# mazrk7/gmvae

Hardware: AMD Instinct MI355X
Metric: ELBO-samples/sec (higher is better)
Workload: dtype f32; 1 GPU; gmvae train step (noise+fwd+bwd+allreduce+TF-Adam), D=784 K=10 L=64 hidden=[64] S=1, batch 1024/GPU x 1 GPU (BASELINE configs[2]); global_batch=1024, parallelism=dp1, hipgraph=True, input_pipeline_on_device=False, safe_schedule=False

## Files before the change

gmvae_amd/csrc/mega2.hpp:

```cpp
#pragma once
#include "mega.hpp"

namespace gmvae {

struct M2 {
  static constexpr int H = 64, L = 64, K = 10, KP = 16, L2 = 128, D = 784, K2 = 12;
  static constexpr int NT = D / 16;
  static constexpr int DC = 16 * kM2ProdTiles;
  static constexpr int b_y0 = 0, b_y1 = 64, b_g0 = 80, b_p = 144, b_g1 = 272, b_d0 = 400;
  static constexpr int Wy1f = 512;
  static constexpr int Wg0yf = Wy1f + 1024;
  static constexpr int Wpf = Wg0yf + 1024;
  static constexpr int imgF_early = Wpf + 2048;
  static constexpr int Wg1f = imgF_early;
  static constexpr int Wd0f = Wg1f + 8192;
  static constexpr int imgF = Wd0f + 4096;
  static constexpr int Wd0b = 0;
  static constexpr int Wg1b = Wd0b + 4096;
  static constexpr int Wg0yb = Wg1b + 8192;
  static constexpr int Wpb = Wg0yb + 1024;
  static constexpr int Wy1b = Wpb + 2048;
  static constexpr int imgB = Wy1b + 1024;
  static constexpr int dF = 0, dFq = 16 * DC * 4;
  static constexpr int dB = 4 * dFq, dBq = (DC / 4) * 64 * 4;
  static constexpr int dbias = dB + 4 * dBq, dbq = DC;
  static constexpr int dimg = dbias + 4 * dbq;
  static constexpr int ld64 = 68, ld128 = 132, ldk = 20;
  static constexpr int IMG = 0;
  static constexpr int P_h1 = IMG + imgF;
  static constexpr int P_y = P_h1 + 16 * ld128;
  static constexpr int P_hg = P_y + 16 * ldk;
  static constexpr int P_pp = P_hg + 16 * ld64;
  static constexpr int P_qp = P_pp + 16 * ld128;
  static constexpr int P_z = P_qp + 16 * ld128;
  static constexpr int P_sp = P_z + 16 * ld64;
  static constexpr int P_hd = P_sp + 16 * 64;
  static constexpr int P_eps = P_hd + 16 * ld64;
  static constexpr int P_u = P_eps + 16 * 64;
  static constexpr int P_lg = P_u + 256;
  static constexpr int nll = P_lg + 16 * ldk;
  static constexpr int rsum = nll + 64;
  static constexpr int red = rsum + 128;
  static constexpr int dred = red + 2048;
  static constexpr int P_dhd = dred + 8192;
  static constexpr int total = P_dhd + 16 * ld64;
  static constexpr int P_dz = dred;
  static constexpr int P_dqp = P_dz + 16 * ld64;
  static constexpr int P_dpp = P_dqp + 16 * ld128;
  static constexpr int P_dhg = P_dpp + 16 * ld128;
  static constexpr int P_dl = P_dhg + 16 * ld64;
  static_assert(P_dl + 16 * ldk <= P_dhd, "backward panels must fit the dred region");
  static_assert(total * 4 <= 160 * 1024, "LDS budget");
  static constexpr int fl_kq = 196, fl_W = imgF, fl_A = fl_W + fl_kq * 64;
  static_assert(fl_A + 32 * kFlLda <= total, "first-layer staging must fit");
  static constexpr int imgF_pieces = (imgF + 2047) / 2048;
};

template <int KT, int NPAD>
__device__ __forceinline__ f32x4 m2_tile(const float* __restrict__ Wimg, const int nt, const float* __restrict__ Pin,
                                         const int ld, const int kt0, const int ln, const int lk, f32x4 acc) {
  float4 a[KT], b[KT];
#pragma unroll
  for (int t = 0; t < KT; ++t) {
    a[t] = *reinterpret_cast<const float4*>(Wimg + ((((kt0 + t) * 4 + lk) * NPAD + nt * 16 + ln) << 2));
    b[t] = *reinterpret_cast<const float4*>(Pin + ln * ld + (kt0 + t) * 16 + 4 * lk);
  }
#pragma unroll
  for (int t = 0; t < KT; ++t) {
    acc = __builtin_amdgcn_mfma_f32_16x16x4f32(a[t].x, b[t].x, acc, 0, 0, 0);
    acc = __builtin_amdgcn_mfma_f32_16x16x4f32(a[t].y, b[t].y, acc, 0, 0, 0);
    acc = __builtin_amdgcn_mfma_f32_16x16x4f32(a[t].z, b[t].z, acc, 0, 0, 0);
    acc = __builtin_amdgcn_mfma_f32_16x16x4f32(a[t].w, b[t].w, acc, 0, 0, 0);
  }
  return acc;
}
__device__ __forceinline__ void granule_publish(unsigned long long* p, const unsigned long long v) {
  __hip_atomic_store(p, v, __ATOMIC_RELAXED, __HIP_MEMORY_SCOPE_AGENT);
}
typedef unsigned u32x4_t __attribute__((ext_vector_type(4)));
__device__ __forceinline__ void granule2_publish(unsigned long long* p, const unsigned epoch, const float v0, const float v1) {
  const u32x4_t t = {__float_as_uint(v0), epoch, __float_as_uint(v1), epoch};
  asm volatile("global_store_dwordx4 %0, %1, off sc1\n\ts_nop 1" ::"v"(p), "v"(t) : "memory");
}
__device__ __forceinline__ u32x4_t granule2_load(const unsigned long long* p) {
  u32x4_t r;
  asm volatile("global_load_dwordx4 %0, %1, off sc1" : "=v"(r) : "v"(p) : "memory");
  return r;
}
#ifndef M2_L2_SWEEPS
#define M2_L2_SWEEPS 0
#endif
__device__ __forceinline__ u32x4_t granule2_load_l2(const unsigned long long* p) {
  u32x4_t r;
  asm volatile("global_load_dwordx4 %0, %1, off sc0" : "=v"(r) : "v"(p) : "memory");
  return r;
}
template <int N>
__device__ __forceinline__ void g2_wait(u32x4_t (&v)[N]) {
  static_assert(N == 6 || N == 8, "operand lists below");
  if constexpr (N == 8)
    asm volatile("s_waitcnt vmcnt(0)" : "+v"(v[0]), "+v"(v[1]), "+v"(v[2]), "+v"(v[3]), "+v"(v[4]), "+v"(v[5]), "+v"(v[6]), "+v"(v[7])::"memory");
  else
    asm volatile("s_waitcnt vmcnt(0)" : "+v"(v[0]), "+v"(v[1]), "+v"(v[2]), "+v"(v[3]), "+v"(v[4]), "+v"(v[5])::"memory");
}
__device__ __forceinline__ float4 f4(const f32x4 v) { return make_float4(v[0], v[1], v[2], v[3]); }
__device__ __forceinline__ float4 ld4(const float* p) { return *reinterpret_cast<const float4*>(p); }
__device__ __forceinline__ void st4(float* p, const float4 v) { *reinterpret_cast<float4*>(p) = v; }
__device__ __forceinline__ void st1o(float* p, const float v) {
  __hip_atomic_store(reinterpret_cast<unsigned*>(p), __float_as_uint(v), __ATOMIC_RELAXED, __HIP_MEMORY_SCOPE_AGENT);
}

template <int FUSE>
__device__ __forceinline__ int mega2_body(const MegaArgs& a, float* const sm, unsigned* const m3_flags = nullptr) {
  constexpr int H = M2::H, L = M2::L, K = M2::K, D = M2::D, L2 = M2::L2, K2 = M2::K2;
  constexpr int Q = 4, H2f = 2 * H;
  const int tid = threadIdx.x, lane = tid & 63, wave = __builtin_amdgcn_readfirstlane(tid >> 6);
  const int ln = lane & 15, lk = lane >> 4;
  const int B = a.B, nP = ((B + kPanel - 1) / kPanel + 1) & ~1;
  const int bid = blockIdx.x;
  const int q = bid < nP * (Q - 1) ? 1 + bid / nP : 0;
  const int pnl = bid < nP * (Q - 1) ? bid % nP : bid - nP * (Q - 1);
  const int r0 = pnl * kPanel;
  const int nrow = min(kPanel, B - r0);
  const bool lead = q == 0;
  const bool act = FUSE ? q == 1 : lead;
  if (a.span && tid == 0) a.span[2 * bid] = wall_clock64();
#define M2_SPAN_END() if (!FUSE && a.span && threadIdx.x == 0) a.span[2 * blockIdx.x + 1] = wall_clock64()
  const unsigned spin_limit = *a.err_word ? 0u : (1u << 19);
  const unsigned epoch0 = *a.epoch_word;
  float* const img = sm + M2::IMG;
  float *P_h1 = sm + M2::P_h1, *P_y = sm + M2::P_y, *P_hg = sm + M2::P_hg, *P_pp = sm + M2::P_pp, *P_qp = sm + M2::P_qp;
  float *P_z = sm + M2::P_z, *P_sp = sm + M2::P_sp, *P_hd = sm + M2::P_hd, *P_eps = sm + M2::P_eps, *P_u = sm + M2::P_u;
  float *P_lg = sm + M2::P_lg, *nllp = sm + M2::nll, *rsum = sm + M2::rsum, *red = sm + M2::red, *dred = sm + M2::dred;
  float* P_dhd = sm + M2::P_dhd;
  GMVAE_STAMP(0);
#define M2_WC(i) if (a.dbg && a.fine == 5 && threadIdx.x == 0) a.dbg[(size_t)blockIdx.x * 16 + 8 + (i)] = wall_clock64()
#define M2_FC(i) if (a.dbg && a.fine == 6 && threadIdx.x == 0) a.dbg[(size_t)blockIdx.x * 16 + 8 + (i)] = __builtin_amdgcn_s_memtime()

  float flt[4] = {0.f, 0.f, 0.f, 0.f};
  {
    constexpr int KQ = M2::fl_kq, kq4 = KQ / 4;
    float* const Wst = sm + M2::fl_W;
    float* const A_x = sm + M2::fl_A;
    const int k0 = q * KQ;
    const int sp = pnl >> 1, hh = pnl & 1;
    const int rs0 = sp * 2 * kPanel;
    const float* const W0 = (hh ? a.w0b : a.w0a) + (long long)k0 * H;
    const unsigned epoch_fl = epoch0;
    const unsigned long long step = a.step_dev[0];
    constexpr int qer = L / 4, qur = (K + 3) / 4, qe = kPanel * qer, qu = kPanel * qur;
    float nz[4] = {0.f, 0.f, 0.f, 0.f};
    f32x4 acc = {0.f, 0.f, 0.f, 0.f};
    unsigned xw[4];
    const int row_ = lane >> 4, piece = lane & 15;
    const int src = row_ * 64 + ((piece ^ ((row_ & 1) << 2)) << 2);
#pragma unroll
    for (int j = 0; j < 3; ++j) {
      const int idx = wave + 8 * j;
      __builtin_amdgcn_global_load_lds(W0 + (idx << 8) + src, Wst + (idx << 8), 16, 0, 0);
    }
#pragma unroll
    for (int it = 0; it < 4; ++it) {
      const int i = min(tid + it * kMT, 2 * kPanel * kq4 - 1);
      const int row = i / kq4, k4 = (i - row * kq4) * 4;
      const unsigned wv = *reinterpret_cast<const unsigned*>(a.x + (long long)min(rs0 + row, B - 1) * D + k0 + k4);
      xw[it] = rs0 + row < B ? wv : 0u;
    }
#pragma unroll
    for (int j = 0; j < 4; ++j) {
      const int idx = 24 + min(wave + 8 * j, 24);
      __builtin_amdgcn_global_load_lds(W0 + (idx << 8) + src, Wst + (idx << 8), 16, 0, 0);
    }
#pragma unroll
    for (int j = 0; j < M2::imgF_pieces; ++j) {
      const int c = min(wave * 256 + j * 2048, M2::imgF - 256);
      __builtin_amdgcn_global_load_lds(a.img2f + c + lane * 4, img + c, 16, 0, 0);
    }
    M2_FC(0);
    if (tid < qe + qu && nrow > 0) {
      const bool is_u = tid >= qe;
      const int li = is_u ? tid - qe : tid;
      const int qpr = is_u ? qur : qer;
      const int row = li / qpr, quad = li - row * qpr;
      noise_vals(a.row0 + (unsigned long long)(r0 + row), (unsigned)quad, is_u, a.seed, step, nz);
    }
    static_assert(M2::imgF_pieces == 9, "the counted waits below assume 9 image pieces per wave");
    asm volatile("s_waitcnt vmcnt(13)" ::: "memory");
    M2_FC(1);
#pragma unroll
    for (int it = 0; it < 4; ++it) {
      const int i = tid + it * kMT;
      if (i < 2 * kPanel * kq4) {
        const int row = i / kq4, k4 = (i - row * kq4) * 4;
        const unsigned w = xw[it];
        float2* const dst = reinterpret_cast<float2*>(A_x + row * kFlLda + k4);
        dst[0] = make_float2((float)(w & 0xff), (float)((w >> 8) & 0xff));
        dst[1] = make_float2((float)((w >> 16) & 0xff), (float)(w >> 24));
      }
    }
    __syncthreads();
    M2_FC(2);
    const int tl = wave & 3, rt = wave >> 2;
    const int swz = ((tl * 16 + ln) ^ ((lk & 1) << 4)) - (tl * 16 + ln);
    const float* const Wt = Wst + swz;
    const float* const At = A_x + rt * kPanel * kFlLda;
    acc = tile_ksteps<1, kFlLda>(At, Wt, H, 1, tl, 0, 24, 24, lane, acc);
    M2_FC(3);
    asm volatile("s_waitcnt vmcnt(9)" ::: "memory");
    __syncthreads();
    M2_FC(4);
    acc = tile_ksteps<1, kFlLda>(At, Wt, H, 1, tl, 24, 49, 49, lane, acc);
    constexpr int ngr = 2 * kPanel * H;
    {
      unsigned long long* xo = a.xfl + (((long long)sp * 4 + q) * 2 + hh) * ngr;
      granule2_publish(xo + ((wave * 2 + 0) * 64 + lane) * 2, epoch_fl, acc[0], acc[1]);
      granule2_publish(xo + ((wave * 2 + 1) * 64 + lane) * 2, epoch_fl, acc[2], acc[3]);
    }
    M2_FC(5);
    if (bid == 0 && tid == 0) a.step_dev[1] = step;
    if (nrow <= 0) {
      asm volatile("s_waitcnt vmcnt(0)" ::: "memory");
      M2_SPAN_END();
      return 0;
    }
    M2_WC(5);
    __syncthreads();
    if (tid < qe) {
      st4(P_eps + tid * 4, make_float4(nz[0], nz[1], nz[2], nz[3]));
    } else if (tid < qe + qu) {
      const int li = tid - qe, row = li / qur, k0u = (li - row * qur) * 4;
#pragma unroll
      for (int j = 0; j < 4; ++j)
        if (k0u + j < K) P_u[row * 16 + k0u + j] = nz[j];
    }
    {
      const unsigned long long* const xp0 = a.xfl + ((long long)sp * 4 * 2 + (wave >> 2)) * ngr + (((hh * 4 + (wave & 3)) * 2) * 64 + lane) * 2;
      u32x4_t gv[8];
      unsigned spins = 0;
      for (;;) {
        if (M2_L2_SWEEPS > 0 && spins < M2_L2_SWEEPS && (wave >> 2) == hh) {
#pragma unroll
          for (int pq = 0; pq < 4; ++pq) {
            gv[2 * pq] = granule2_load_l2(xp0 + (long long)pq * 2 * ngr);
            gv[2 * pq + 1] = granule2_load_l2(xp0 + (long long)pq * 2 * ngr + 128);
          }
        } else {
#pragma unroll
          for (int pq = 0; pq < 4; ++pq) {
            gv[2 * pq] = granule2_load(xp0 + (long long)pq * 2 * ngr);
            gv[2 * pq + 1] = granule2_load(xp0 + (long long)pq * 2 * ngr + 128);
          }
        }
        g2_wait(gv);
        bool ok = true;
#pragma unroll
        for (int i = 0; i < 8; ++i) ok = ok && gv[i][1] == epoch_fl && gv[i][3] == epoch_fl;
        if (__all(ok)) break;
        if (++spins > spin_limit) {
          if (lane == 0) atomicExch(a.err_word, 1u);
#pragma unroll
          for (int i = 0; i < 8; ++i) { gv[i][0] = 0x7fc00000u; gv[i][2] = 0x7fc00000u; }
          break;
        }
        __builtin_amdgcn_s_sleep(2);
      }
#pragma unroll
      for (int r = 0; r < 4; ++r) {
        flt[r] = __uint_as_float(gv[0 + (r >> 1)][2 * (r & 1)]);
        flt[r] += __uint_as_float(gv[2 + (r >> 1)][2 * (r & 1)]);
        flt[r] += __uint_as_float(gv[4 + (r >> 1)][2 * (r & 1)]);
        flt[r] += __uint_as_float(gv[6 + (r >> 1)][2 * (r & 1)]);
      }
      if (a.dbg && a.fine >= 5 && tid == 0) {
        a.dbg[(size_t)blockIdx.x * 16 + 14] = spins;
        a.dbg[(size_t)blockIdx.x * 16 + 0] = __builtin_amdgcn_s_getreg((3 << 11) | 20) & 15u;
      }
    }
  }
  M2_WC(6);
  M2_FC(6);
  const int ntq = m2_dec_ntiles(q);
  const bool two = wave + 8 < ntq;
  const bool one = wave < ntq;
  float4 wf[2][4], wb[2][4], bias4[2];
  unsigned xb[2] = {0u, 0u};
  {
    const float* const dfq = a.dimg2 + M2::dF + q * M2::dFq;
    const float* const dbq = a.dimg2 + M2::dB + q * M2::dBq;
    const float* const bq = a.dimg2 + M2::dbias + q * M2::dbq;
#pragma unroll
    for (int it = 0; it < 2; ++it) {
      if (it == 0 ? one : two) {
        const int lt = wave + 8 * it;
#pragma unroll
        for (int kt = 0; kt < 4; ++kt) wf[it][kt] = ld4(dfq + (((kt * 4 + lk) * M2::DC + lt * 16 + ln) << 2));
#pragma unroll
        for (int ht = 0; ht < 4; ++ht) wb[it][ht] = ld4(dbq + (((lt * 4 + lk) * 64 + ht * 16 + ln) << 2));
        bias4[it] = ld4(bq + lt * 16 + 4 * lk);
        const int c0 = m2_dec_tile(q, lt) * 16;
        xb[it] = *reinterpret_cast<const unsigned*>(a.x + (long long)min(r0 + ln, B - 1) * D + c0 + 4 * lk);
      }
    }
  }
  if (two) asm volatile("s_waitcnt vmcnt(20)" ::: "memory");
  else if (one) asm volatile("s_waitcnt vmcnt(10)" ::: "memory");
  else asm volatile("s_waitcnt vmcnt(0)" ::: "memory");
  __syncthreads();
  M2_FC(7);
  {
#pragma unroll
    for (int r = 0; r < 4; ++r) {
      const int row = lk * 4 + r, col = wave * 16 + ln;
      if (col < H) {
        const float h = fmaxf(flt[r] + img[M2::b_y0 + col], 0.f);
        P_h1[row * M2::ld128 + col] = h;
      } else {
        P_h1[row * M2::ld128 + col] = flt[r];
      }
    }
  }
  __syncthreads();
  GMVAE_STAMP(1);
  if (act && tid < 256) {
    const int row = tid >> 4, c = (tid & 15) << 2;
    if (row < nrow) st4o(a.hy1 + (long long)(r0 + row) * H + c, ld4(P_h1 + row * M2::ld128 + c));
  }
  if (wave < 4) {
    f32x4 acc = {0.f, 0.f, 0.f, 0.f};
    acc = m2_tile<1, 16>(img + M2::Wy1f, 0, P_h1, M2::ld128, wave, ln, lk, acc);
    st4(red + wave * 320 + ln * M2::ldk + 4 * lk, f4(acc));
  }
  __syncthreads();
  if (tid < 256) {
    const int row = tid >> 4, k = tid & 15;
    const bool ok = row < nrow, kv = k < K;
    float lg = -INFINITY, av = -INFINITY;
    if (kv) {
      lg = red[row * M2::ldk + k] + red[320 + row * M2::ldk + k] + red[640 + row * M2::ldk + k] + red[960 + row * M2::ldk + k] +
           img[M2::b_y1 + k];
      const float uu = ok ? P_u[row * 16 + k] : 0.5f;
      av = (lg - flog(-flog(uu))) * a.invT;
    }
    const float mx = row16_max(av);
    const float se = row16_sum(kv ? fexp(av - mx) : 0.f);
    const float lse = mx + flog(se);
    const float lga[1] = {lg};
    float lpa[1];
    cat_log_softmax<Row16, 1>(lga, lpa);
    float yv = 0.f, ne = 0.f;
    if (kv) {
      yv = fexp(av - lse);
      const float lp = lpa[0];
      P_lg[row * M2::ldk + k] = lp;
      ne = fexp(lp) * lp;
      if (ok && act) st1o(a.y + (long long)(r0 + row) * K2 + k, yv);
    }
    P_y[row * M2::ldk + k] = yv;
    ne = row16_sum(ne);
    if (k == 0) { nllp[3 * kPanel + row] = ne; if (ok && lead) st1o(a.nent + r0 + row, ne); }
  }
  __syncthreads();
  GMVAE_STAMP(2);
  {
    f32x4 acc = {0.f, 0.f, 0.f, 0.f};
    acc = m2_tile<1, 128>(img + M2::Wpf, wave, P_y, M2::ldk, 0, ln, lk, acc);
    const int c0 = wave * 16 + 4 * lk;
    const float4 bb = ld4(img + M2::b_p + c0);
    st4(P_pp + ln * M2::ld128 + c0, make_float4(acc[0] + bb.x, acc[1] + bb.y, acc[2] + bb.z, acc[3] + bb.w));
    if (wave < 4) {
      f32x4 ac2 = {0.f, 0.f, 0.f, 0.f};
      ac2 = m2_tile<1, 64>(img + M2::Wg0yf, wave, P_y, M2::ldk, 0, ln, lk, ac2);
      const float4 gx = ld4(P_h1 + ln * M2::ld128 + H + c0), bg = ld4(img + M2::b_g0 + c0);
      const float4 h = make_float4(fmaxf(ac2[0] + gx.x + bg.x, 0.f), fmaxf(ac2[1] + gx.y + bg.y, 0.f),
                                   fmaxf(ac2[2] + gx.z + bg.z, 0.f), fmaxf(ac2[3] + gx.w + bg.w, 0.f));
      st4(P_hg + ln * M2::ld64 + c0, h);
      if (act && ln < nrow) st4o(a.hg1 + (long long)(r0 + ln) * H + c0, h);
    }
  }
  __syncthreads();
  {
    f32x4 acc = {0.f, 0.f, 0.f, 0.f};
    acc = m2_tile<4, 128>(img + M2::Wg1f, wave, P_hg, M2::ld64, 0, ln, lk, acc);
    const int c0 = wave * 16 + 4 * lk;
    const float4 bb = ld4(img + M2::b_g1 + c0);
    st4(P_qp + ln * M2::ld128 + c0, make_float4(acc[0] + bb.x, acc[1] + bb.y, acc[2] + bb.z, acc[3] + bb.w));
  }
  __syncthreads();
  GMVAE_STAMP(3);
  {
    const int row = tid >> 5, sub = tid & 31;
    const bool ok = row < nrow;
    float aq = 0.f, ap = 0.f;
#pragma unroll
    for (int l = sub; l < L; l += 32) {
      float* const qr = P_qp + row * M2::ld128;
      float* const pr = P_pp + row * M2::ld128;
      const float mu = qr[l];
      const float vq = qr[L + l] + a.c;
      float sgq;
      const float sg = fmaxf(softplus_sig(vq, sgq), a.smin);
      const float ee = ok ? P_eps[row * 64 + l] : 0.f;
      const float zz = mu + sg * ee;
      P_z[row * M2::ld64 + l] = zz;
      qr[l] = sgq;
      qr[L + l] = sg;
      aq += -0.5f * ee * ee - 0.5f * kLog2Pi - flog(sg);
      const float vp = pr[L + l] + a.c;
      float sgp;
      const float sp = fmaxf(softplus_sig(vp, sgp), a.smin);
      const float t = (zz - pr[l]) * __builtin_amdgcn_rcpf(sp);
      ap += -0.5f * t * t - 0.5f * kLog2Pi - flog(sp);
      pr[l] = t;
      pr[L + l] = sp;
      P_sp[row * 64 + l] = sgp;
    }
    aq = row32_sum(aq); ap = row32_sum(ap);
    if (sub == 0) {
      nllp[row] = aq; nllp[kPanel + row] = ap;
      if (ok && lead) { st1o(a.logq + r0 + row, aq); st1o(a.logp + r0 + row, ap); }
    }
  }
  __syncthreads();
  if (act && tid >= 256) {
    const int t2 = tid - 256, row = t2 >> 4, c = (t2 & 15) << 2;
    if (row < nrow) st4o(a.z + (long long)(r0 + row) * L + c, ld4(P_z + row * M2::ld64 + c));
  }
  if (wave < 4) {
    f32x4 acc = {0.f, 0.f, 0.f, 0.f};
    acc = m2_tile<4, 64>(img + M2::Wd0f, wave, P_z, M2::ld64, 0, ln, lk, acc);
    const int c0 = wave * 16 + 4 * lk;
    const float4 bb = ld4(img + M2::b_d0 + c0);
    const float4 h = make_float4(fmaxf(acc[0] + bb.x, 0.f), fmaxf(acc[1] + bb.y, 0.f), fmaxf(acc[2] + bb.z, 0.f), fmaxf(acc[3] + bb.w, 0.f));
    st4(P_hd + ln * M2::ld64 + c0, h);
    if (act && ln < nrow) st4o(a.hd1 + (long long)(r0 + ln) * H + c0, h);
  }
  __syncthreads();
  GMVAE_STAMP(4);
  if (lead) dma_copy_m(img, a.img2b, M2::imgB, wave, lane);

  f32x4 dacc[4];
#pragma unroll
  for (int ht = 0; ht < 4; ++ht) dacc[ht] = f32x4{0.f, 0.f, 0.f, 0.f};
  float rs = 0.f;
  float4 gkeep[2];
  {
    float4 hb[4];
#pragma unroll
    for (int kt = 0; kt < 4; ++kt) hb[kt] = ld4(P_hd + ln * M2::ld64 + kt * 16 + 4 * lk);
#pragma unroll
    for (int it = 0; it < 2; ++it) {
      const int lt = wave + 8 * it;
      if (lt < ntq) {
        f32x4 acc = {0.f, 0.f, 0.f, 0.f};
#pragma unroll
        for (int kt = 0; kt < 4; ++kt) {
          acc = __builtin_amdgcn_mfma_f32_16x16x4f32(wf[it][kt].x, hb[kt].x, acc, 0, 0, 0);
          acc = __builtin_amdgcn_mfma_f32_16x16x4f32(wf[it][kt].y, hb[kt].y, acc, 0, 0, 0);
          acc = __builtin_amdgcn_mfma_f32_16x16x4f32(wf[it][kt].z, hb[kt].z, acc, 0, 0, 0);
          acc = __builtin_amdgcn_mfma_f32_16x16x4f32(wf[it][kt].w, hb[kt].w, acc, 0, 0, 0);
        }
        const float bv[4] = {bias4[it].x, bias4[it].y, bias4[it].z, bias4[it].w};
        const bool ok = ln < nrow;
        float g[4];
#pragma unroll
        for (int r = 0; r < 4; ++r) {
          const float lam = acc[r] + bv[r] + a.gen_bias;
          const float e = fexp(-fabsf(lam));
          const float rcp = __builtin_amdgcn_rcpf(1.f + e);
          const float sp = fmaxf(lam, 0.f) - flog(rcp);
          const float sgm = lam >= 0.f ? rcp : e * rcp;
          const float x_ = ok ? (float)((xb[it] >> (8 * r)) & 0xffu) : 0.f;
          rs += ok ? x_ * lam - sp : 0.f;
          g[r] = ok ? sgm - x_ : 0.f;
        }
        if (lead) gkeep[it] = make_float4(g[0], g[1], g[2], g[3]);
        else if (ok) st4o(a.g + (long long)(r0 + ln) * D + m2_dec_tile(q, lt) * 16 + 4 * lk, make_float4(g[0], g[1], g[2], g[3]));
#pragma unroll
        for (int ht = 0; ht < 4; ++ht) {
          dacc[ht] = __builtin_amdgcn_mfma_f32_16x16x4f32(wb[it][ht].x, g[0], dacc[ht], 0, 0, 0);
          dacc[ht] = __builtin_amdgcn_mfma_f32_16x16x4f32(wb[it][ht].y, g[1], dacc[ht], 0, 0, 0);
          dacc[ht] = __builtin_amdgcn_mfma_f32_16x16x4f32(wb[it][ht].z, g[2], dacc[ht], 0, 0, 0);
          dacc[ht] = __builtin_amdgcn_mfma_f32_16x16x4f32(wb[it][ht].w, g[3], dacc[ht], 0, 0, 0);
        }
      }
    }
  }
  GMVAE_STAMP(5);
  rs += __shfl_xor(rs, 16, 64);
  rs += __shfl_xor(rs, 32, 64);
  if (lk == 0) rsum[wave * kPanel + ln] = rs;
#pragma unroll
  for (int ht = 0; ht < 4; ++ht) st4(dred + wave * 1024 + (((ht * 4 + lk) * 16 + ln) << 2), f4(dacc[ht]));
  __syncthreads();
  M2_WC(0);
  const unsigned epoch = epoch0;
  constexpr int ngr = kPanel * H + kPanel;
  float4 dsum = make_float4(0.f, 0.f, 0.f, 0.f);
  float rsn = 0.f;
  if (tid < 256) {
#pragma unroll
    for (int w = 0; w < kMW; ++w) {
      const float4 o = ld4(dred + w * 1024 + 4 * tid);
      dsum.x += o.x; dsum.y += o.y; dsum.z += o.z; dsum.w += o.w;
    }
  } else if (tid < 256 + kPanel) {
#pragma unroll
    for (int w = 0; w < kMW; ++w) rsn += rsum[w * kPanel + (tid - 256)];
  }
  const int orow = tid & 15, ocol = (tid >> 4) << 2;
  if (!lead) {
    unsigned long long* xo = a.xchg + ((long long)pnl * (Q - 1) + (q - 1)) * ngr;
    if (tid < 256) {
      granule2_publish(xo + ((wave * 2 + 0) * 64 + lane) * 2, epoch, dsum.x, dsum.y);
      granule2_publish(xo + ((wave * 2 + 1) * 64 + lane) * 2, epoch, dsum.z, dsum.w);
    } else if (tid < 256 + kPanel) {
      granule_publish(xo + kPanel * H + (tid - 256), ((unsigned long long)epoch << 32) | __float_as_uint(rsn));
    }
    M2_WC(1);
    if (!FUSE && bid == 0 && tid == 0 && a.lr_t_out) {
      const double t = (double)(a.step_dev[0] + 1ull);
      *a.lr_t_out = (float)((double)a.lr * sqrt(1.0 - pow((double)a.b2, t)) / (1.0 - pow((double)a.b1, t)));
    }
    M2_SPAN_END();
    return 1;
  }
  M2_WC(1);
  {
    const unsigned long long* xi = a.xchg + (long long)pnl * (Q - 1) * ngr;
    const bool wd = tid < 256, wn = tid >= 256 && tid < 256 + kPanel;
    unsigned spins = 0;
    if (wave < 4) {
      u32x4_t v[6];
      const unsigned long long* const xs = xi + ((wave * 2) * 64 + lane) * 2;
      for (;;) {
        if (M2_L2_SWEEPS > 0 && spins < M2_L2_SWEEPS) {
#pragma unroll
          for (int pq = 0; pq < Q - 1; ++pq) {
            v[2 * pq] = granule2_load_l2(xs + (long long)pq * ngr);
            v[2 * pq + 1] = granule2_load_l2(xs + (long long)pq * ngr + 128);
          }
        } else {
#pragma unroll
          for (int pq = 0; pq < Q - 1; ++pq) {
            v[2 * pq] = granule2_load(xs + (long long)pq * ngr);
            v[2 * pq + 1] = granule2_load(xs + (long long)pq * ngr + 128);
          }
        }
        g2_wait(v);
        bool ok = true;
#pragma unroll
        for (int i = 0; i < 6; ++i) ok = ok && v[i][1] == epoch && v[i][3] == epoch;
        if (__all(ok)) break;
        if (++spins > spin_limit) {
          if (lane == 0) atomicExch(a.err_word, 1u);
#pragma unroll
          for (int i = 0; i < 6; ++i) { v[i][0] = 0x7fc00000u; v[i][2] = 0x7fc00000u; }
          break;
        }
        __builtin_amdgcn_s_sleep(4);
      }
#pragma unroll
      for (int pq = 0; pq < Q - 1; ++pq) {
        dsum.x += __uint_as_float(v[2 * pq][0]); dsum.y += __uint_as_float(v[2 * pq][2]);
        dsum.z += __uint_as_float(v[2 * pq + 1][0]); dsum.w += __uint_as_float(v[2 * pq + 1][2]);
      }
    } else if (wave == 4) {
      unsigned long long v[Q - 1];
      const unsigned long long* const xs = xi + kPanel * H + min(lane, kPanel - 1);
      for (;;) {
#pragma unroll
        for (int pq = 0; pq < Q - 1; ++pq)
          v[pq] = (M2_L2_SWEEPS > 0 && spins < M2_L2_SWEEPS) ? __hip_atomic_load(xs + (long long)pq * ngr, __ATOMIC_RELAXED, __HIP_MEMORY_SCOPE_WORKGROUP)
                                                             : __hip_atomic_load(xs + (long long)pq * ngr, __ATOMIC_RELAXED, __HIP_MEMORY_SCOPE_AGENT);
        __builtin_amdgcn_sched_barrier(0);
        bool ok = true;
#pragma unroll
        for (int pq = 0; pq < Q - 1; ++pq) ok = ok && (unsigned)(v[pq] >> 32) == epoch;
        if (__all(ok)) break;
        if (++spins > spin_limit) {
          if (lane == 0) atomicExch(a.err_word, 1u);
#pragma unroll
          for (int pq = 0; pq < Q - 1; ++pq) v[pq] = 0x7fc00000ull;
          break;
        }
        __builtin_amdgcn_s_sleep(4);
      }
#pragma unroll
      for (int pq = 0; pq < Q - 1; ++pq)
        if (wn) rsn += __uint_as_float((unsigned)v[pq]);
    }
    if (a.dbg && a.fine >= 5 && tid == 0) a.dbg[(size_t)blockIdx.x * 16 + 15] = spins;
    if (ln < nrow && one) {
      st4o(a.g + (long long)(r0 + ln) * D + m2_dec_tile(0, wave) * 16 + 4 * lk, gkeep[0]);
      if (two) st4o(a.g + (long long)(r0 + ln) * D + m2_dec_tile(0, wave + 8) * 16 + 4 * lk, gkeep[1]);
    }
    M2_WC(2);
    if (wd) {
      const float4 hd = ld4(P_hd + orow * M2::ld64 + ocol);
      const bool ok = orow < nrow;
      const float4 d = make_float4((ok && hd.x > 0.f) ? dsum.x : 0.f, (ok && hd.y > 0.f) ? dsum.y : 0.f,
                                   (ok && hd.z > 0.f) ? dsum.z : 0.f, (ok && hd.w > 0.f) ? dsum.w : 0.f);
      st4(P_dhd + orow * M2::ld64 + ocol, d);
      if (ok) st4o(a.dhd1 + (long long)(r0 + orow) * H + ocol, d);
    }
    if (wn) {
      const int row = tid - 256;
      if (row < nrow) {
        st1o(a.logpx + r0 + row, rsn);
        st1o(a.logw + r0 + row, rsn + nllp[kPanel + row] - nllp[row] - nllp[3 * kPanel + row]);
      }
    }
  }
  M2_WC(3);
  if (wave > 4) { if (one) asm volatile("s_waitcnt vmcnt(1)" ::: "memory"); else asm volatile("s_waitcnt vmcnt(0)" ::: "memory"); }
  __syncthreads();
  M2_WC(4);
  GMVAE_STAMP(6);
  float *P_dz = sm + M2::P_dz, *P_dqp = sm + M2::P_dqp, *P_dpp = sm + M2::P_dpp, *P_dhg = sm + M2::P_dhg, *P_dl = sm + M2::P_dl;
  if (wave < 4) {
    f32x4 acc = {0.f, 0.f, 0.f, 0.f};
    acc = m2_tile<4, 64>(img + M2::Wd0b, wave, P_dhd, M2::ld64, 0, ln, lk, acc);
    st4(P_dz + ln * M2::ld64 + wave * 16 + 4 * lk, f4(acc));
  }
  __syncthreads();
  {
    const int row = tid >> 5, sub = tid & 31;
    const bool ok = row < nrow;
#pragma unroll
    for (int l = sub; l < L; l += 32) {
      float dmu = 0.f, draw = 0.f, dmup = 0.f, drawp = 0.f;
      if (ok) {
        const float sg = P_qp[row * M2::ld128 + L + l];
        const float sp = P_pp[row * M2::ld128 + L + l], t = P_pp[row * M2::ld128 + l];
        const float isp = __builtin_amdgcn_rcpf(sp);
        const float pterm = t * isp;
        dmup = -pterm;
        drawp = (sp > a.smin) ? (1.f - t * t) * isp * P_sp[row * 64 + l] : 0.f;
        dmu = P_dz[row * M2::ld64 + l] + pterm;
        const float dsg = dmu * P_eps[row * 64 + l] - __builtin_amdgcn_rcpf(sg);
        draw = (sg > a.smin) ? dsg * P_qp[row * M2::ld128 + l] : 0.f;
      }
      P_dqp[row * M2::ld128 + l] = dmu;
      P_dqp[row * M2::ld128 + L + l] = draw;
      P_dpp[row * M2::ld128 + l] = dmup;
      P_dpp[row * M2::ld128 + L + l] = drawp;
    }
  }
  __syncthreads();
  {
    const int row = tid >> 5, c = (tid & 31) << 2;
    if (row < nrow) {
      st4o(a.dqp + (long long)(r0 + row) * L2 + c, ld4(P_dqp + row * M2::ld128 + c));
      st4o(a.dpp + (long long)(r0 + row) * L2 + c, ld4(P_dpp + row * M2::ld128 + c));
    }
  }
  {
    const int t = wave & 3, kh = wave >> 2;
    f32x4 acc = {0.f, 0.f, 0.f, 0.f};
    acc = m2_tile<4, 64>(img + M2::Wg1b, t, P_dqp, M2::ld128, 4 * kh, ln, lk, acc);
    if (kh) st4(red + t * 256 + ((lk * 16 + ln) << 2), f4(acc));
    __syncthreads();
    if (!kh) {
      const float4 o = ld4(red + t * 256 + ((lk * 16 + ln) << 2));
      const int c0 = t * 16 + 4 * lk;
      const float4 hg = ld4(P_hg + ln * M2::ld64 + c0);
      const bool ok = ln < nrow;
      const float4 d = make_float4((ok && hg.x > 0.f) ? acc[0] + o.x : 0.f, (ok && hg.y > 0.f) ? acc[1] + o.y : 0.f,
                                   (ok && hg.z > 0.f) ? acc[2] + o.z : 0.f, (ok && hg.w > 0.f) ? acc[3] + o.w : 0.f);
      st4(P_dhg + ln * M2::ld64 + c0, d);
      if (ok) st4o(a.dhg1 + (long long)(r0 + ln) * H + c0, d);
    }
  }
  __syncthreads();
  {
    f32x4 acc = {0.f, 0.f, 0.f, 0.f};
    if (wave < 4) {
      acc = m2_tile<1, 16>(img + M2::Wg0yb, 0, P_dhg, M2::ld64, wave, ln, lk, acc);
      acc = m2_tile<1, 16>(img + M2::Wpb, 0, P_dpp, M2::ld128, 4 + wave, ln, lk, acc);
    } else {
      acc = m2_tile<1, 16>(img + M2::Wpb, 0, P_dpp, M2::ld128, wave - 4, ln, lk, acc);
    }
    st4(red + wave * 256 + ((lk * 16 + ln) << 2), f4(acc));
  }
  __syncthreads();
  if (tid < 256) {
    const int row = tid >> 4, k = tid & 15;
    const bool ok = row < nrow, kv = k < K && ok;
    float dy = 0.f;
#pragma unroll
    for (int w = 0; w < kMW; ++w) dy += red[w * 256 + (((k >> 2) * 16 + row) << 2) + (k & 3)];
    const float ya[1] = {kv ? P_y[row * M2::ldk + k] : 0.f}, dya[1] = {kv ? dy : 0.f};
    float daa[1];
    cat_softmax_bwd<Row16, 1>(ya, dya, daa);
    const float ne = nllp[3 * kPanel + row];
    float dl = 0.f;
    if (kv) {
      const float lp = P_lg[row * M2::ldk + k];
      dl = daa[0] * a.invT + fexp(lp) * (lp - ne);
      st1o(a.dlogits + (long long)(r0 + row) * K2 + k, dl);
    }
    P_dl[row * M2::ldk + k] = dl;
  }
  __syncthreads();
  if (wave < 4) {
    f32x4 acc = {0.f, 0.f, 0.f, 0.f};
    acc = m2_tile<1, 64>(img + M2::Wy1b, wave, P_dl, M2::ldk, 0, ln, lk, acc);
    const int c0 = wave * 16 + 4 * lk;
    const float4 hy = ld4(P_h1 + ln * M2::ld128 + c0);
    if (ln < nrow)
      st4o(a.dhy1 + (long long)(r0 + ln) * H + c0,
           make_float4(hy.x > 0.f ? acc[0] : 0.f, hy.y > 0.f ? acc[1] : 0.f, hy.z > 0.f ? acc[2] : 0.f, hy.w > 0.f ? acc[3] : 0.f));
  }
  GMVAE_STAMP(7);
  M2_SPAN_END();
#undef M2_SPAN_END
  return 2;
}

__global__ __launch_bounds__(kMT) void mega2_fwd_bwd(const MegaArgs a) {
  extern __shared__ __attribute__((aligned(16))) float sm[];
  mega2_body<0>(a, sm);
}

}
```

Before: 32.56 million samples/sec.

## Repartition first-layer GEMM by output column tile with in-block K reduction

The first encoder layer is redistributed so each block owns one 16-column output tile across the full input depth. The four K-quarters are reduced inside the block through LDS, and only one pre-summed tile per block is published. Raw uint8 input bytes are loaded straight into LDS and unpacked inside the MFMA loop, replacing the register load and float conversion pass. Cross-block polling now reads two granules per wave instead of eight, and the block's own tile is taken from LDS, cutting global traffic and spin latency at the cost of a new LDS reduction and barrier.

After: 31.91 million samples/sec. 2.0% lower.

```diff
diff --git a/gmvae_amd/csrc/mega2.hpp b/gmvae_amd/csrc/mega2.hpp
--- a/gmvae_amd/csrc/mega2.hpp
+++ b/gmvae_amd/csrc/mega2.hpp
@@ -51,8 +51,14 @@
   static constexpr int P_dl = P_dhg + 16 * ld64;
   static_assert(P_dl + 16 * ldk <= P_dhd, "backward panels must fit the dred region");
   static_assert(total * 4 <= 160 * 1024, "LDS budget");
-  static constexpr int fl_kq = 196, fl_W = imgF, fl_A = fl_W + fl_kq * 64;
-  static_assert(fl_A + 32 * kFlLda <= total, "first-layer staging must fit");
+  static constexpr int fl_kq = 196, fl_k1 = 96, fl_k2 = fl_kq - fl_k1, fl_xp = 13, fl_xld = 4 * fl_xp;
+  static constexpr int fl_W = imgF, fl_W2 = fl_W + 4 * fl_k1 * 16, fl_A = fl_W + D * 16;
+  static constexpr int fl_xpieces = 4 * 32 * fl_xp;
+  static constexpr int fl_Z = fl_A + fl_xpieces * 4, fl_R = fl_Z + 64;
+  static_assert(fl_k1 % 16 == 0 && (4 * fl_k2) % 16 == 0 && fl_xpieces % 64 == 0, "whole bursts");
+  static_assert(16 * (fl_xp - 1) <= fl_kq && fl_kq <= 16 * fl_xp && fl_kq % 4 == 0, "x pieces of a quarter");
+  static_assert(fl_R >= P_u + 256 && fl_R >= dred && fl_R + 8 * 256 <= P_dhd, "the accumulators outlive the staging: clear of P_eps, P_u");
+  static_assert(fl_R + 8 * 256 <= total, "first-layer staging must fit");
   static constexpr int imgF_pieces = (imgF + 2047) / 2048;
 };
 
@@ -97,8 +103,10 @@
 }
 template <int N>
 __device__ __forceinline__ void g2_wait(u32x4_t (&v)[N]) {
-  static_assert(N == 6 || N == 8, "operand lists below");
-  if constexpr (N == 8)
+  static_assert(N == 2 || N == 6 || N == 8, "operand lists below");
+  if constexpr (N == 2)
+    asm volatile("s_waitcnt vmcnt(0)" : "+v"(v[0]), "+v"(v[1])::"memory");
+  else if constexpr (N == 8)
     asm volatile("s_waitcnt vmcnt(0)" : "+v"(v[0]), "+v"(v[1]), "+v"(v[2]), "+v"(v[3]), "+v"(v[4]), "+v"(v[5]), "+v"(v[6]), "+v"(v[7])::"memory");
   else
     asm volatile("s_waitcnt vmcnt(0)" : "+v"(v[0]), "+v"(v[1]), "+v"(v[2]), "+v"(v[3]), "+v"(v[4]), "+v"(v[5])::"memory");
@@ -139,37 +147,40 @@
 
   float flt[4] = {0.f, 0.f, 0.f, 0.f};
   {
-    constexpr int KQ = M2::fl_kq, kq4 = KQ / 4;
     float* const Wst = sm + M2::fl_W;
-    float* const A_x = sm + M2::fl_A;
-    const int k0 = q * KQ;
+    unsigned* const Xst = reinterpret_cast<unsigned*>(sm + M2::fl_A);
+    float* const Rq = sm + M2::fl_R;
     const int sp = pnl >> 1, hh = pnl & 1;
+    const int ct = hh * 4 + q;
     const int rs0 = sp * 2 * kPanel;
-    const float* const W0 = (hh ? a.w0b : a.w0a) + (long long)k0 * H;
+    const float* const W0 = (hh ? a.w0b : a.w0a) + q * 16 + ((lane & 3) << 2);
     const unsigned epoch_fl = epoch0;
     const unsigned long long step = a.step_dev[0];
     constexpr int qer = L / 4, qur = (K + 3) / 4, qe = kPanel * qer, qu = kPanel * qur;
     float nz[4] = {0.f, 0.f, 0.f, 0.f};
     f32x4 acc = {0.f, 0.f, 0.f, 0.f};
-    unsigned xw[4];
-    const int row_ = lane >> 4, piece = lane & 15;
-    const int src = row_ * 64 + ((piece ^ ((row_ & 1) << 2)) << 2);
+    const int wr = lane >> 2;
 #pragma unroll
     for (int j = 0; j < 3; ++j) {
       const int idx = wave + 8 * j;
-      __builtin_amdgcn_global_load_lds(W0 + (idx << 8) + src, Wst + (idx << 8), 16, 0, 0);
-    }
-#pragma unroll
-    for (int it = 0; it < 4; ++it) {
-      const int i = min(tid + it * kMT, 2 * kPanel * kq4 - 1);
-      const int row = i / kq4, k4 = (i - row * kq4) * 4;
-      const unsigned wv = *reinterpret_cast<const unsigned*>(a.x + (long long)min(rs0 + row, B - 1) * D + k0 + k4);
-      xw[it] = rs0 + row < B ? wv : 0u;
+      const int R = idx * 16 + wr, kq = R / M2::fl_k1;
+      __builtin_amdgcn_global_load_lds(W0 + (kq * M2::fl_kq + (R - kq * M2::fl_k1)) * H, Wst + (idx << 8), 16, 0, 0);
     }
 #pragma unroll
     for (int j = 0; j < 4; ++j) {
-      const int idx = 24 + min(wave + 8 * j, 24);
-      __builtin_amdgcn_global_load_lds(W0 + (idx << 8) + src, Wst + (idx << 8), 16, 0, 0);
+      const int idx = min(wave + 8 * j, M2::fl_xpieces / 64 - 1);
+      const int pc = idx * 64 + lane;
+      const int rw = pc / M2::fl_xp, j13 = pc - rw * M2::fl_xp;
+      const int kq = rw >> 5, row = rw & 31;
+      const unsigned char* const src = a.x + (long long)min(rs0 + row, B - 1) * D + kq * M2::fl_kq +
+                                       (j13 < M2::fl_xp - 1 ? 16 * j13 : M2::fl_kq - 16);
+      __builtin_amdgcn_global_load_lds(reinterpret_cast<const unsigned*>(src), Xst + (idx << 8), 16, 0, 0);
+    }
+#pragma unroll
+    for (int j = 0; j < 4; ++j) {
+      const int idx = min(wave + 8 * j, 24);
+      const int R = idx * 16 + wr, kq = R / M2::fl_k2;
+      __builtin_amdgcn_global_load_lds(W0 + (kq * M2::fl_kq + M2::fl_k1 + (R - kq * M2::fl_k2)) * H, sm + M2::fl_W2 + (idx << 8), 16, 0, 0);
     }
 #pragma unroll
     for (int j = 0; j < M2::imgF_pieces; ++j) {
@@ -177,6 +188,7 @@
       __builtin_amdgcn_global_load_lds(a.img2f + c + lane * 4, img + c, 16, 0, 0);
     }
     M2_FC(0);
+    if (tid < M2::fl_xp) st4(sm + M2::fl_Z + tid * 4, make_float4(0.f, 0.f, 0.f, 0.f));
     if (tid < qe + qu && nrow > 0) {
       const bool is_u = tid >= qe;
       const int li = is_u ? tid - qe : tid;
@@ -187,34 +199,48 @@
     static_assert(M2::imgF_pieces == 9, "the counted waits below assume 9 image pieces per wave");
     asm volatile("s_waitcnt vmcnt(13)" ::: "memory");
     M2_FC(1);
-#pragma unroll
-    for (int it = 0; it < 4; ++it) {
-      const int i = tid + it * kMT;
-      if (i < 2 * kPanel * kq4) {
-        const int row = i / kq4, k4 = (i - row * kq4) * 4;
-        const unsigned w = xw[it];
-        float2* const dst = reinterpret_cast<float2*>(A_x + row * kFlLda + k4);
-        dst[0] = make_float2((float)(w & 0xff), (float)((w >> 8) & 0xff));
-        dst[1] = make_float2((float)((w >> 16) & 0xff), (float)(w >> 24));
-      }
-    }
     __syncthreads();
     M2_FC(2);
-    const int tl = wave & 3, rt = wave >> 2;
-    const int swz = ((tl * 16 + ln) ^ ((lk & 1) << 4)) - (tl * 16 + ln);
-    const float* const Wt = Wst + swz;
-    const float* const At = A_x + rt * kPanel * kFlLda;
-    acc = tile_ksteps<1, kFlLda>(At, Wt, H, 1, tl, 0, 24, 24, lane, acc);
+    const int kq = wave & 3, rt = wave >> 2;
+    const unsigned* const xr = rs0 + rt * kPanel + ln < B ? Xst + ((kq * 32 + rt * kPanel + ln) * M2::fl_xld)
+                                                          : reinterpret_cast<const unsigned*>(sm + M2::fl_Z);
+    const unsigned sh = 8u * lk;
+    const float* const w1 = Wst + (kq * M2::fl_k1 + lk) * 16 + ln;
+    const float* const w2 = sm + M2::fl_W2 + (kq * M2::fl_k2 + lk) * 16 + ln;
+#define M2_FL8(XP, WP)                                                                                             \
+    {                                                                                                              \
+      const u32x4_t xa = *reinterpret_cast<const u32x4_t*>(XP), xb_ = *reinterpret_cast<const u32x4_t*>((XP) + 4); \
+      float bv[8];                                                                                                 \
+      _Pragma("unroll") for (int j = 0; j < 8; ++j) bv[j] = (WP)[j * 64];                                           \
+      _Pragma("unroll") for (int j = 0; j < 8; ++j) {                                                               \
+        const unsigned xw_ = j < 4 ? xa[j & 3] : xb_[j & 3];                                                       \
+        acc = __builtin_amdgcn_mfma_f32_16x16x4f32((float)((xw_ >> sh) & 0xffu), bv[j], acc, 0, 0, 0);             \
+      }                                                                                                            \
+    }
+#pragma unroll
+    for (int g8 = 0; g8 < 3; ++g8) M2_FL8(xr + 8 * g8, w1 + g8 * 512)
     M2_FC(3);
     asm volatile("s_waitcnt vmcnt(9)" ::: "memory");
     __syncthreads();
     M2_FC(4);
-    acc = tile_ksteps<1, kFlLda>(At, Wt, H, 1, tl, 24, 49, 49, lane, acc);
-    constexpr int ngr = 2 * kPanel * H;
-    {
-      unsigned long long* xo = a.xfl + (((long long)sp * 4 + q) * 2 + hh) * ngr;
-      granule2_publish(xo + ((wave * 2 + 0) * 64 + lane) * 2, epoch_fl, acc[0], acc[1]);
-      granule2_publish(xo + ((wave * 2 + 1) * 64 + lane) * 2, epoch_fl, acc[2], acc[3]);
+#pragma unroll
+    for (int g8 = 0; g8 < 3; ++g8) M2_FL8(xr + 24 + 8 * g8, w2 + g8 * 512)
+#undef M2_FL8
+    acc = __builtin_amdgcn_mfma_f32_16x16x4f32((float)((xr[M2::fl_xld - 1] >> sh) & 0xffu), w2[24 * 64], acc, 0, 0, 0);
+    st4(Rq + ((wave * 64 + lane) << 2), f4(acc));
+    __syncthreads();
+    constexpr int ngr = 2 * kPanel * 16;
+    if (wave < 2) {
+      const float* const rp = Rq + ((wave * 4 * 64 + lane) << 2);
+      float4 o = ld4(rp);
+#pragma unroll
+      for (int pq = 1; pq < 4; ++pq) {
+        const float4 t = ld4(rp + pq * 256);
+        o.x += t.x; o.y += t.y; o.z += t.z; o.w += t.w;
+      }
+      unsigned long long* xo = a.xfl + ((long long)sp * 8 + ct) * ngr + wave * (ngr / 2);
+      granule2_publish(xo + (0 * 64 + lane) * 2, epoch_fl, o.x, o.y);
+      granule2_publish(xo + (1 * 64 + lane) * 2, epoch_fl, o.z, o.w);
     }
     M2_FC(5);
     if (bid == 0 && tid == 0) a.step_dev[1] = step;
@@ -224,7 +250,6 @@
       return 0;
     }
     M2_WC(5);
-    __syncthreads();
     if (tid < qe) {
       st4(P_eps + tid * 4, make_float4(nz[0], nz[1], nz[2], nz[3]));
     } else if (tid < qe + qu) {
@@ -234,44 +259,36 @@
         if (k0u + j < K) P_u[row * 16 + k0u + j] = nz[j];
     }
     {
-      const unsigned long long* const xp0 = a.xfl + ((long long)sp * 4 * 2 + (wave >> 2)) * ngr + (((hh * 4 + (wave & 3)) * 2) * 64 + lane) * 2;
-      u32x4_t gv[8];
       unsigned spins = 0;
-      for (;;) {
-        if (M2_L2_SWEEPS > 0 && spins < M2_L2_SWEEPS && (wave >> 2) == hh) {
-#pragma unroll
-          for (int pq = 0; pq < 4; ++pq) {
-            gv[2 * pq] = granule2_load_l2(xp0 + (long long)pq * 2 * ngr);
-            gv[2 * pq + 1] = granule2_load_l2(xp0 + (long long)pq * 2 * ngr + 128);
+      if (wave == ct) {
+        const float* const rp = Rq + ((hh * 4 * 64 + lane) << 2);
+        float4 o = ld4(rp);
+#pragma unroll
+        for (int pq = 1; pq < 4; ++pq) {
+          const float4 t = ld4(rp + pq * 256);
+          o.x += t.x; o.y += t.y; o.z += t.z; o.w += t.w;
+        }
+        flt[0] = o.x; flt[1] = o.y; flt[2] = o.z; flt[3] = o.w;
+      } else {
+        const unsigned long long* const xp0 = a.xfl + ((long long)sp * 8 + wave) * ngr + hh * (ngr / 2) + lane * 2;
+        u32x4_t gv[2];
+        for (;;) {
+          gv[0] = granule2_load(xp0);
+          gv[1] = granule2_load(xp0 + 128);
+          g2_wait(gv);
+          const bool ok = gv[0][1] == epoch_fl && gv[0][3] == epoch_fl && gv[1][1] == epoch_fl && gv[1][3] == epoch_fl;
+          if (__all(ok)) break;
+          if (++spins > spin_limit) {
+            if (lane == 0) atomicExch(a.err_word, 1u);
+            gv[0][0] = gv[0][2] = gv[1][0] = gv[1][2] = 0x7fc00000u;
+            break;
           }
-        } else {
-#pragma unroll
-          for (int pq = 0; pq < 4; ++pq) {
-            gv[2 * pq] = granule2_load(xp0 + (long long)pq * 2 * ngr);
-            gv[2 * pq + 1] = granule2_load(xp0 + (long long)pq * 2 * ngr + 128);
-          }
+          __builtin_amdgcn_s_sleep(2);
         }
-        g2_wait(gv);
-        bool ok = true;
-#pragma unroll
-        for (int i = 0; i < 8; ++i) ok = ok && gv[i][1] == epoch_fl && gv[i][3] == epoch_fl;
-        if (__all(ok)) break;
-        if (++spins > spin_limit) {
-          if (lane == 0) atomicExch(a.err_word, 1u);
-#pragma unroll
-          for (int i = 0; i < 8; ++i) { gv[i][0] = 0x7fc00000u; gv[i][2] = 0x7fc00000u; }
-          break;
-        }
-        __builtin_amdgcn_s_sleep(2);
-      }
-#pragma unroll
-      for (int r = 0; r < 4; ++r) {
-        flt[r] = __uint_as_float(gv[0 + (r >> 1)][2 * (r & 1)]);
-        flt[r] += __uint_as_float(gv[2 + (r >> 1)][2 * (r & 1)]);
-        flt[r] += __uint_as_float(gv[4 + (r >> 1)][2 * (r & 1)]);
-        flt[r] += __uint_as_float(gv[6 + (r >> 1)][2 * (r & 1)]);
-      }
-      if (a.dbg && a.fine >= 5 && tid == 0) {
+        flt[0] = __uint_as_float(gv[0][0]); flt[1] = __uint_as_float(gv[0][2]);
+        flt[2] = __uint_as_float(gv[1][0]); flt[3] = __uint_as_float(gv[1][2]);
+      }
+      if (a.dbg && a.fine >= 5 && lane == 0 && wave == (ct == 0 ? 1 : 0) && (wave == 0 || a.fine == 5)) {
         a.dbg[(size_t)blockIdx.x * 16 + 14] = spins;
         a.dbg[(size_t)blockIdx.x * 16 + 0] = __builtin_amdgcn_s_getreg((3 << 11) | 20) & 15u;
       }
```
